# huster-wgm/SRCGAN

Hardware: AMD Instinct MI355X
Metric: paired SR-CycleGAN train images/sec at x4 256->1024 (higher is better)
Workload: dtype bf16; 1 GPU; Sat2Aerx4 paired G+D step (BASELINE configs[1]): 23-block RRDB generator + 3-layer PatchGAN, 3x256x256->3x1024x1024, batch 16/GPU; per_gpu_batch=16, global_batch=16, parallelism=dp1, gradient_exchange=none (1 rank)

## Files before the change

include/srcgan_amd.h:

```cpp
#ifndef SRCGAN_AMD_H
#define SRCGAN_AMD_H

#include <stddef.h>
#include <stdint.h>

#ifdef __cplusplus
extern "C" {
#endif

#define SRCGAN_F32 0
#define SRCGAN_BF16 1
#define SRCGAN_F16 2

int srcgan_version(void);
const char* srcgan_last_error(void);
int srcgan_dtype_size(int dtype);

int srcgan_nchw_f32_to_nhwc(const float* src, void* dst, int B, int C, int H, int W,
                            int cs, int dtype, void* stream);
int srcgan_nhwc_to_nchw_f32(const void* src, float* dst, int B, int C, int H, int W,
                            int cs, int coff, int dtype, void* stream);

size_t srcgan_packed_weight_bytes(int rows, int kdim, int ntaps, int dtype);
int srcgan_pack_weight(const float* w, void* wp, int rows, int kdim, int tys, int txs,
// ... 34 lines not shown
    int nsplit;
    long sr, sk, sty, stx, off;
    float alpha;
    int accumulate;
} srcgan_wgrad_desc;
size_t srcgan_conv_wgrad_slab_bytes(int Cout, int Cin, int kh, int kw, int nsplit);
int srcgan_conv_wgrad_nsplit(int B, int OH, int OW, int Cout, int Cin, int stride);
int srcgan_conv_wgrad(const srcgan_wgrad_desc* d, void* stream);

typedef struct srcgan_wgrad_seg { int g0, g1; float* grad; float* bias; int Cin; float alpha; } srcgan_wgrad_seg;
typedef struct srcgan_wgrad_dense_desc {
    const void* dy; const void* x; float* slab;
    int dtype;
    int B, H, W;
    int G, dy_cs, dy_coff;
    int C, x_cs, x_coff;
    int nseg;
    srcgan_wgrad_seg seg[8];
    int accumulate;
    long dy_plane, x_plane;
} srcgan_wgrad_dense_desc;
size_t srcgan_wgrad_dense_slab_bytes(int G, int C, int dtype, int B, int H, int W);
int srcgan_wgrad_dense(const srcgan_wgrad_dense_desc* d, void* stream);

int srcgan_col_reduce_blocks(long npix);
int srcgan_col_reduce(int mode, const void* a, int a_cs, int a_coff, const void* z, int z_cs, int z_coff,
                      const float* m, const float* rstd, long npix, int C, float scale,
                      float* out0, float* out1, float* scratch, int dtype, void* stream);

int srcgan_bn_finalize(const float* mean, const float* var, float* rstd, float* running_mean,
                       float* running_var, int64_t* num_batches_tracked, int C, long count,
                       float momentum, float eps, void* stream);
int srcgan_bn_eval_rstd(const float* running_var, float* rstd, int C, float eps, void* stream);
int srcgan_bn_apply_lrelu(const void* z, void* y, const float* mean, const float* rstd, const float* gamma,
                          const float* beta, long npix, int C, int cs, float slope, int dtype, void* stream);
int srcgan_bn_bwd_apply(const void* g, const void* z, void* dz, const float* mean, const float* rstd,
                        const float* gamma, const float* sum_g, const float* sum_gx, long npix, int C, int cs,
                        int dtype, void* stream);

int srcgan_add_inplace(void* y, int y_cs, int y_coff, const void* x, int x_cs, int x_coff,
                       const void* mz, int mz_cs, int mz_coff, float mslope, long npix, int C, int dtype, void* stream);
int srcgan_add_inplace_planes(void* y, int y_cs, int y_coff, long y_plane, const void* x, int x_cs, int x_coff, long x_plane,
                              const void* mz, int mz_cs, int mz_coff, long mz_plane, float mslope, long npix, int C,
                              int dtype, void* stream);

size_t srcgan_gn_scratch_floats(int B, int C);
// ... 382 lines not shown
```

srcgan_amd/_native.py:

```python
from __future__ import annotations

import ctypes as C
import os
from typing import Optional, Sequence

import torch

_HERE = os.path.dirname(os.path.abspath(__file__))
LIB_PATH = os.environ.get("SRCGAN_AMD_LIB") or os.path.join(_HERE, "lib", "libsrcgan_amd.so")

F32, BF16, F16 = 0, 1, 2
_DTYPES = {"fp32": F32, "f32": F32, "float32": F32, torch.float32: F32,
           "bf16": BF16, "bfloat16": BF16, torch.bfloat16: BF16,
           "fp16": F16, "f16": F16, "float16": F16, "half": F16, torch.float16: F16, F32: F32, BF16: BF16, F16: F16}
_default_dtype = _DTYPES[os.environ.get("SRCGAN_AMD_DTYPE", "fp32")]


def dtype_id(d) -> int:
    if d is None:
        return _default_dtype
    try:
        return _DTYPES[d]
    except KeyError:
        raise ValueError(f"unsupported compute dtype {d!r} (use 'fp32', 'bf16' or 'fp16')") from None
# ... 25 lines not shown
                ("sign_out", C.c_void_p), ("sign_in", C.c_void_p), ("npar", C.c_int), ("wpar_stride", C.c_long)]


class WgradDesc(C.Structure):
    _fields_ = [("dy", C.c_void_p), ("x", C.c_void_p), ("slab", C.c_void_p), ("grad", C.c_void_p), ("bias_grad", C.c_void_p),
                ("dtype", C.c_int), ("kh", C.c_int), ("kw", C.c_int), ("stride", C.c_int),
                ("B", C.c_int), ("H", C.c_int), ("W", C.c_int), ("Cin", C.c_int), ("x_cs", C.c_int), ("x_coff", C.c_int),
                ("OH", C.c_int), ("OW", C.c_int), ("Cout", C.c_int), ("dy_cs", C.c_int), ("dy_coff", C.c_int),
                ("pad_y", C.c_int), ("pad_x", C.c_int), ("nsplit", C.c_int),
                ("sr", C.c_long), ("sk", C.c_long), ("sty", C.c_long), ("stx", C.c_long), ("off", C.c_long),
                ("alpha", C.c_float), ("accumulate", C.c_int)]


class WgradSeg(C.Structure):
    _fields_ = [("g0", C.c_int), ("g1", C.c_int), ("grad", C.c_void_p), ("bias", C.c_void_p), ("Cin", C.c_int), ("alpha", C.c_float)]


class WgradDenseDesc(C.Structure):
    _fields_ = [("dy", C.c_void_p), ("x", C.c_void_p), ("slab", C.c_void_p), ("dtype", C.c_int),
                ("B", C.c_int), ("H", C.c_int), ("W", C.c_int),
                ("G", C.c_int), ("dy_cs", C.c_int), ("dy_coff", C.c_int),
                ("C", C.c_int), ("x_cs", C.c_int), ("x_coff", C.c_int),
                ("nseg", C.c_int), ("seg", WgradSeg * 8), ("accumulate", C.c_int), ("dy_plane", C.c_long), ("x_plane", C.c_long)]


class RddbCfg(C.Structure):
    _fields_ = [("in_ch", C.c_int), ("out_ch", C.c_int), ("up", C.c_int), ("nf", C.c_int), ("nb", C.c_int), ("gc", C.c_int),
                ("B", C.c_int), ("H", C.c_int), ("W", C.c_int), ("dtype", C.c_int), ("down", C.c_int), ("legacy", C.c_int)]


class NetOpts(C.Structure):
    _fields_ = [("wpack", C.c_void_p), ("pack", C.c_int), ("rrdb_lo", C.c_int), ("rrdb_hi", C.c_int), ("guard", C.c_void_p)]


class ResDeconvCfg(C.Structure):
    _fields_ = [("in_ch", C.c_int), ("out_ch", C.c_int), ("B", C.c_int), ("H", C.c_int), ("W", C.c_int), ("dtype", C.c_int),
                ("layers", C.c_int * 4), ("norm", C.c_int)]


class SrNetCfg(C.Structure):
    _fields_ = [(n, C.c_int) for n in ("kind", "in_ch", "out_ch", "up", "base", "B", "H", "W", "dtype", "nres")]


class SrDenseCfg(C.Structure):
    _fields_ = [(n, C.c_int) for n in ("kind", "in_ch", "out_ch", "B", "H", "W", "dtype", "growth", "num_blocks", "num_layers", "up")]

# ... 32 lines not shown


class NLayerDCfg(C.Structure):
    _fields_ = [("in_ch", C.c_int), ("ndf", C.c_int), ("n_layers", C.c_int),
                ("B", C.c_int), ("H", C.c_int), ("W", C.c_int), ("dtype", C.c_int), ("training", C.c_int), ("norm", C.c_int)]


_P, _I, _L, _F, _S = C.c_void_p, C.c_int, C.c_long, C.c_float, C.c_size_t
SIGNATURES = {
    "srcgan_version": (_I, []),
    "srcgan_last_error": (C.c_char_p, []),
    "srcgan_dtype_size": (_I, [_I]),
    "srcgan_nchw_f32_to_nhwc": (_I, [_P, _P, _I, _I, _I, _I, _I, _I, _P]),
    "srcgan_nhwc_to_nchw_f32": (_I, [_P, _P, _I, _I, _I, _I, _I, _I, _I, _P]),
    "srcgan_packed_weight_bytes": (_S, [_I, _I, _I, _I]),
    "srcgan_pack_weight": (_I, [_P, _P, _I, _I, _I, _I, _L, _L, _L, _L, _L, _I, _P]),
    "srcgan_pack_weight_part": (_I, [_P, _P, _I, _I, _I, _I, _L, _L, _L, _L, _L, _I, _I, _F, _I, _P]),
    "srcgan_conv_igemm": (_I, [C.POINTER(ConvDesc), _P]),
    "srcgan_conv_wgrad_slab_bytes": (_S, [_I, _I, _I, _I, _I]),
    "srcgan_conv_wgrad_nsplit": (_I, [_I, _I, _I, _I, _I, _I]),
    "srcgan_conv_wgrad": (_I, [C.POINTER(WgradDesc), _P]),
    "srcgan_wgrad_dense_slab_bytes": (_S, [_I, _I, _I, _I, _I, _I]),
    "srcgan_wgrad_dense": (_I, [C.POINTER(WgradDenseDesc), _P]),
    "srcgan_col_reduce_blocks": (_I, [_L]),
    "srcgan_col_reduce": (_I, [_I, _P, _I, _I, _P, _I, _I, _P, _P, _L, _I, _F, _P, _P, _P, _I, _P]),
    "srcgan_bn_finalize": (_I, [_P, _P, _P, _P, _P, _P, _I, _L, _F, _F, _P]),
    "srcgan_bn_eval_rstd": (_I, [_P, _P, _I, _F, _P]),
    "srcgan_bn_apply_lrelu": (_I, [_P, _P, _P, _P, _P, _P, _L, _I, _I, _F, _I, _P]),
    "srcgan_bn_bwd_apply": (_I, [_P, _P, _P, _P, _P, _P, _P, _P, _L, _I, _I, _I, _P]),
    "srcgan_add_inplace": (_I, [_P, _I, _I, _P, _I, _I, _P, _I, _I, _F, _L, _I, _I, _P]),
    "srcgan_add_inplace_planes": (_I, [_P, _I, _I, _L, _P, _I, _I, _L, _P, _I, _I, _L, _F, _L, _I, _I, _P]),
    "srcgan_gn_scratch_floats": (_S, [_I, _I]),
    "srcgan_gn_forward": (_I, [_P, _I, _P, _I, _P, _I, _P, _P, _P, _I, _L, _I, _I, _F, _I, _F, _I, _P, _P]),
    "srcgan_gn_backward": (_I, [_P, _I, _P, _I, _P, _I, _P, _P, _P, _I, _P, _I, _I, _P, _P, _I, _F, _I, _L, _I, _I, _I, _P, _P]),
    "srcgan_ca_scratch_floats": (_S, [_I, _L, _I]),
    "srcgan_ca_forward": (_I, [_P, _I, _P, _I, _P, _I, _P, _P, _P, _P, _P, _I, _L, _I, _I, _I, _P, _P]),
    "srcgan_ca_backward": (_I, [_P, _I, _P, _I, _P, _P, _P, _P, _I, _P, _I, _I, _P, _P, _P, _P, _I, _L, _I, _I, _I, _P, _P]),
    "srcgan_s2d_shift": (_I, [_P, _I, _P, _I, _I, _I, _I, _I, _I, _I, _I, _I, _I, _P]),
    "srcgan_d2s_shift": (_I, [_P, _I, _P, _I, _I, _I, _I, _I, _I, _I, _I, _I, _I, _I, _P]),
    "srcgan_prelu_forward": (_I, [_P, _I, _P, _P, _P, _I, _F, _P, _I, _I, _I, _I, _I, _I, _I, _I, _I, _I, _P]),
    "srcgan_prelu_scratch_floats": (_S, [_I, _I, _I, _I, _I]),
    "srcgan_prelu_backward": (_I, [_P, _I, _P, _I, _P, _P, _P, _I, _P, _I, _F, _I, _P, _P, _I, _I, _I, _I, _I, _I, _I, _I, _I, _P, _P]),
    "srcgan_reflect_pad_nhwc": (_I, [_P, _I, _P, _I, _I, _I, _I, _I, _I, _I, _P]),
    "srcgan_reflect_pad_bwd_nhwc": (_I, [_P, _I, _P, _I, _I, _I, _I, _I, _I, _I, _I, _P]),
    "srcgan_tanh_forward": (_I, [_P, _I, _P, _I, _L, _I, _I, _P]),
    "srcgan_tanh_backward": (_I, [_P, _I, _P, _I, _P, _I, _L, _I, _I, _I, _P]),
# ... 195 lines not shown
```

srcgan_amd/build.py:

```python
import glob
import os
import subprocess
import sys
from concurrent.futures import ThreadPoolExecutor

HERE = os.path.dirname(os.path.abspath(__file__))
CSRC = os.path.join(HERE, "csrc")
LIBDIR = os.path.join(HERE, "lib")
LIB = os.path.join(LIBDIR, "libsrcgan_amd.so")
SOURCES = ["conv_entry.hip", "conv_igemm.hip", "conv_par4.hip", "deconv_k3s2.hip", "conv3x3_dma.hip", "conv_wgrad.hip", "wgrad_dense.hip", "elementwise.hip", "class_losses.hip", "groupnorm.hip", "chan_attn.hip", "back_proj.hip", "reflect_pad.hip", "unet_skip.hip", "metrics.hip", "shift_select.hip", "scene_score.hip", "colour.hip", "tiles.hip", "vgg_loss.hip", "nets.hip", "oplist.hip"]
FLAGS = ["--offload-arch=gfx950", "-O3", "-std=c++17", "-fPIC", "-Wall", "-Wno-unused-function"]


def _hipcc():
    for c in (os.environ.get("HIPCC"), "/opt/rocm/bin/hipcc", "hipcc"):
        if c and (os.path.isabs(c) and os.path.exists(c) or not os.path.isabs(c)):
            return c
    raise RuntimeError("hipcc not found")


def _stale(target, deps):
    if not os.path.exists(target):
        return True
    t = os.path.getmtime(target)
    return any(os.path.getmtime(d) > t for d in deps)


def build(force=False, verbose=True):
    os.makedirs(LIBDIR, exist_ok=True)
    hipcc = _hipcc()
    headers = glob.glob(os.path.join(CSRC, "*.h")) + [os.path.join(HERE, "..", "include", "srcgan_amd.h")]
    objs, jobs = [], []
    for s in SOURCES:
# ... 23 lines not shown
```

srcgan_amd/csrc/nets.hip:

```cpp
#include "net_common.h"
#include <map>
#include <mutex>
#include <string>

int sg_zigzag_next() {
    static const bool zig = sg_env("SRCGAN_NO_ZIGZAG") == nullptr;
    static int flip = 0;
    const int rev = flip;
    flip ^= 1;
    return zig ? rev : 0;
}

namespace {
struct PackCache { std::vector<SgPackJob> host; SgPackJob* dev = nullptr; SgPackJob* pinned = nullptr; size_t cap = 0; hipEvent_t staged = nullptr; };
std::map<std::string, PackCache> g_pack_cache;
std::mutex g_pack_mutex;
}

int sg_pack_list_run(const std::vector<SgPackJob>& jobs, long nblk, void* wp_base, int dtype, const char* tag, const void* key_ptr, void* st,
                     const unsigned long long* guard) {
    if (jobs.empty()) return 0;
    int dev = 0;
    SG_HIP(hipGetDevice(&dev));
    char key[112];
    snprintf(key, sizeof(key), "%s:%d:%p:%d:%zu", tag, dev, key_ptr, dtype, jobs.size());
    std::lock_guard<std::mutex> lock(g_pack_mutex);
// ... 118 lines not shown
    for (int s = 0; s < P.nst; ++s) { for (int q = 0; q < 4; ++q) P.w_up_f[s][q] = pk(c->nf, c->nf, 1); P.w_up_d[s] = pk(c->nf, c->nf, 4); }
    P.w_last_f = pk(c->out_ch, c->nf, 9); P.w_last_d = pk(c->nf, P.out_cs, 9);
    for (int k = 0; k < P.nlw; ++k) { P.lw_f[k] = pk(c->nf, c->nf, 9); P.lw_d[k] = pk(c->nf, c->nf, 9); }
    P.w_rdb_d0 = wb.off;
    for (int i = 0; i < nrdb; ++i)
        for (int j = 0; j < 5; ++j) P.w_rdb_d[i * 5 + j] = pk(j == 0 ? c->nf : c->gc, c->nf + (4 - j) * c->gc, 9);
    P.w_rdb_dsz = wb.off - P.w_rdb_d0;
    P.wpack_bytes = wb.off + 256;
    int n = 0;
    P.p_first_w = n++; P.p_first_b = n++;
    P.p_dn0 = n; n += 2 * P.ndn;
    P.p_rdb0 = n; n += c->nb * 30;
    P.p_trunk_w = n++; P.p_trunk_b = n++;
    if (P.family == RDDB_SRDN) n += c->nb * 30;
    P.p_up0 = n;
    if (P.x2_tail) for (int k = 0; k < P.nlw; ++k) { P.p_lg[k] = n; n += 2; }
    else n += P.nst;
    P.p_last_w = n++;
    P.p_last_b = P.x2_tail ? n++ : -1;
    P.nparams = n;
    return 0;
}

struct RddbNames {
    size_t xin = 0, fea0 = 0, dn[5] = {}, T = 0, U[6] = {}, out = 0, tail[16] = {}, wpk = 0, total = 0;
    std::vector<size_t> A;
    size_t home = 0;
    bool rolling = false;
    size_t bm = 0; long bm_bytes = 0;
    size_t um = 0; long um_bytes = 0;
};

static void rddb_train_names(const srcgan_rddbnet_cfg* c, const RddbPlan& P, RddbNames& N) {
    const size_t e = P.esz, B = c->B, nf = c->nf;
    Bump b;
    N.xin = b.take(B * c->H * c->W * P.in_cs * e);
    if (P.ndn) N.fea0 = b.take(B * c->H * c->W * nf * e);
    for (int s = 0; s < P.ndn; ++s) N.dn[s] = b.take(B * (c->H >> (s + 1)) * (c->W >> (s + 1)) * nf * e);
    static const bool no_sign = sg_env("SRCGAN_NO_SIGNMASK") != nullptr || sg_env("SRCGAN_DMA_CFG") != nullptr;
    N.bm_bytes = (!no_sign && sg_is16(c->dtype) && c->gc == 32 && nf % 32 == 0 && P.family != RDDB_LEGACY) ? (long)B * P.Ht * P.Wt * 4 : 0;
    N.bm = align_up((size_t)P.nplane * P.plane_bytes, 256);
    const size_t szA = align_up(N.bm + 4 * (size_t)N.bm_bytes, 256);
    const size_t A0 = b.take(szA * P.ndense);
    N.A.resize(P.ndense);
    for (int r = 0; r < P.ndense; ++r) N.A[r] = A0 + (size_t)r * szA;
    N.T = b.take(B * P.Ht * P.Wt * nf * e);
    for (int s = 0; s <= P.nup; ++s) N.U[s] = b.take(B * (P.Ht << s) * (P.Wt << s) * nf * e);
    if (P.family == RDDB_SRDN) N.U[0] = N.T;
    for (int k = 0; k < P.ntail; ++k) N.tail[k] = b.take(B * P.tail[k].hout * P.tail[k].wout * nf * e);
    N.out = b.take(B * P.HO * P.WO * P.out_cs * e);
    N.um_bytes = (!no_sign && sg_is16(c->dtype) && nf == 64 && P.nst > 0 && P.family == RDDB_PLAIN) ? (long)B * P.HO * P.WO * 8 : 0;
    if (N.um_bytes) N.um = b.take((size_t)N.um_bytes);
    N.wpk = b.off;
    N.total = N.wpk + P.wpack_bytes;
}

static void rddb_infer_names(const srcgan_rddbnet_cfg* c, const RddbPlan& P, RddbNames& N) {
    const size_t e = P.esz, B = c->B, nf = c->nf;
    Bump b;
    N.rolling = true;
    N.xin = b.take(B * c->H * c->W * P.in_cs * e);
    if (P.ndn) {
        const size_t pp0 = b.take(B * c->H * c->W * nf * e);
        const size_t pp1 = P.ndn > 1 ? b.take(B * (c->H >> 1) * (c->W >> 1) * nf * e) : 0;
        N.fea0 = pp0;
        for (int s = 0; s < P.ndn; ++s) N.dn[s] = (s & 1) ? pp0 : pp1;
    }
    const size_t szA = align_up((size_t)P.nplane * P.plane_bytes, 256);
    size_t slot[3] = {0, 0, 0};
    for (int k = 0; k < 3 && k < P.ndense; ++k) slot[k] = b.take(szA);
    N.A.resize(P.ndense);
    int cur = 0, rrdb_in = 0;
    for (int r = 0; r < P.ndense; ++r) {
        if (r % 3 == 0) rrdb_in = cur;
// ... 27 lines not shown
struct RddbBwdPlan {
    size_t dout, dU[6], Pg[3], szP, dfea_dn[5], dxin, slab, colscr, total;
};
static void rddb_bwd_plan(const srcgan_rddbnet_cfg* c, const RddbPlan& P, RddbBwdPlan& Q) {
    const size_t e = P.esz, B = c->B;
    Bump b;
    Q.dout = b.take(B * P.HO * P.WO * P.out_cs * e);
    for (int s = 0; s <= P.nup; ++s) Q.dU[s] = b.take(B * (P.Ht << s) * (P.Wt << s) * c->nf * e);
    if (P.x2_tail) { Q.dU[1] = b.take(B * P.HO * P.WO * c->nf * e); Q.dU[2] = b.take(B * P.HO * P.WO * c->nf * e); }
    Q.szP = align_up((size_t)P.nplane * P.plane_bytes, 256);
    for (int i = 0; i < 3; ++i) Q.Pg[i] = b.take(Q.szP);
    for (int s = 0; s <= P.ndn; ++s) Q.dfea_dn[s] = b.take(B * (c->H >> s) * (c->W >> s) * c->nf * e);
    Q.dxin = b.take(B * c->H * c->W * P.in_cs * e);
    size_t slab = 0;
    auto mx = [&](size_t v) { if (v > slab) slab = v; };
    mx(wgrad_slab(c->B, c->H, c->W, c->nf, P.in_cs, 3, 3, 1));
    for (int k = 0; k < 5; ++k) mx(wgrad_slab(c->B, P.Ht, P.Wt, k < 4 ? c->gc : c->nf, c->nf + k * c->gc, 3, 3, 1));
    mx(wgrad_slab(c->B, P.Ht, P.Wt, c->nf, c->nf, 3, 3, 1));
    for (int s = 0; s < P.nup; ++s) mx(wgrad_slab(c->B, P.Ht << s, P.Wt << s, c->nf, c->nf, 2, 2, 2));
    for (int k = 0; k < P.ntail; ++k) if (P.tail[k].conv) mx(wgrad_slab(c->B, P.tail[k].hout, P.tail[k].wout, c->nf, c->nf, 3, 3, 1));
    for (int s = 0; s < P.ndn; ++s) mx(wgrad_slab(c->B, c->H >> (s + 1), c->W >> (s + 1), c->nf, c->nf, 3, 3, 2));
    mx(wgrad_slab(c->B, P.HO, P.WO, c->out_ch, c->nf, 3, 3, 1));
    mx(srcgan_wgrad_dense_slab_bytes(P.C, P.C, c->dtype, c->B, P.Ht, P.Wt));
    Q.slab = b.take(slab);
    const long maxpix = (long)B * (P.HO > c->H ? P.HO : c->H) * (P.WO > c->W ? P.WO : c->W);
    Q.colscr = b.take((size_t)2 * srcgan_col_reduce_blocks(maxpix) * P.C * sizeof(float));
    Q.total = b.off + 256;
}

}

extern "C" int srcgan_rddbnet_num_params(const srcgan_rddbnet_cfg* c) { RddbPlan P; if (rddb_plan(c, P)) return -1; return P.nparams; }
extern "C" int srcgan_rddbnet_num_rrdb(const srcgan_rddbnet_cfg* c) { RddbPlan P; if (rddb_plan(c, P)) return -1; return P.nrr; }
extern "C" size_t srcgan_rddbnet_wpack_bytes(const srcgan_rddbnet_cfg* c) { RddbPlan P; if (rddb_plan(c, P)) return 0; return P.wpack_bytes; }
extern "C" size_t srcgan_rddbnet_ws_bytes(const srcgan_rddbnet_cfg* c) {
    RddbPlan P; if (rddb_plan(c, P)) return 0;
    RddbNames N; rddb_train_names(c, P, N); return N.total;
}
extern "C" size_t srcgan_rddbnet_infer_ws_bytes(const srcgan_rddbnet_cfg* c) {
    RddbPlan P; if (rddb_plan(c, P)) return 0;
    RddbNames N; rddb_infer_names(c, P, N); return N.total;
}
extern "C" size_t srcgan_rddbnet_bwd_scratch_bytes(const srcgan_rddbnet_cfg* c) {
    RddbPlan P; if (rddb_plan(c, P)) return 0;
    RddbBwdPlan Q; rddb_bwd_plan(c, P, Q); return Q.total;
}
// ... 138 lines not shown
    RddbPlan P;
    SG_TRY(rddb_plan(c, P));
    RddbNames N;
    if (infer) rddb_infer_names(c, P, N); else rddb_train_names(c, P, N);
    return RddbCall(c, P, N, params, ws, opt, st).forward(x_nchw, y_nchw);
}

extern "C" int srcgan_rddbnet_forward_ex(const srcgan_rddbnet_cfg* c, const float* x_nchw, const float* const* params,
                                         void* ws, float* y_nchw, const srcgan_net_opts* opt, void* st) {
    return rddb_forward(c, false, x_nchw, params, ws, y_nchw, opt, st);
}

extern "C" int srcgan_rddbnet_infer(const srcgan_rddbnet_cfg* c, const float* x_nchw, const float* const* params, void* ws,
                                    float* y_nchw, const srcgan_net_opts* opt, void* st) {
    return rddb_forward(c, true, x_nchw, params, ws, y_nchw, opt, st);
}

extern "C" int srcgan_rddbnet_forward(const srcgan_rddbnet_cfg* c, const float* x_nchw, const float* const* params,
                                      void* ws, float* y_nchw, void* st) {
    return srcgan_rddbnet_forward_ex(c, x_nchw, params, ws, y_nchw, nullptr, st);
}

namespace {

struct RddbBwd : RddbCall {
    const RddbBwdPlan& Q;
    char* s8; float* const* grads;
    float* slab; float* colscr;
    const long npix_t;
    RddbBwd(const RddbCall& call, const RddbBwdPlan& Q_, void* scratch, float* const* grads_)
        : RddbCall(call), Q(Q_), s8((char*)scratch), grads(grads_), slab((float*)(s8 + Q_.slab)), colscr((float*)(s8 + Q_.colscr)),
          npix_t((long)B * H * W) {}
    TRef S_(size_t off, int cs) const { return tref(s8 + off, cs); }
    float* G(int idx) const { return grads[idx]; }
    TRef dout() const { return S_(Q.dout, P.out_cs); }
    TRef dU0() const { return S_(Q.dU[0], nf); }
    TRef Pg(int g) const { return tref(s8 + Q.Pg[g], P.kce, 0, P.plane_bytes); }
    int pack_dgrad(bool pack_dx) const;
    int output_plain() const;
    int output_tail() const;
    int trunk_entry() const;
    int rrdb_range(int r_lo, int r_hi) const;
    int input_side(float* dx_nchw) const;
};

int RddbBwd::pack_dgrad(bool pack_dx) const {
// ... 7 lines not shown
    if (P.family != RDDB_SRDN) packs.add(params[P.p_trunk_w], wp + P.w_trunk_d, nf, nf, 3, 3, L);
    SG_TRY(sg_fill_zero_guarded(wp + P.w_rdb_d0, P.w_rdb_dsz, pack_guard(opt), (hipStream_t)st));
    for (int r = 0; r < P.nrr * 3; ++r) {
        const float a5 = (r % 3 == 2) ? 0.04f : 0.2f;
        for (int j = 0; j < 5; ++j) {
            const int rows = j == 0 ? nf : gc, ss = j == 0 ? 0 : nf + (j - 1) * gc, ktot = nf + (4 - j) * gc;
            for (int m = 5; m > j; --m) {
                const int cin_m = nf + (m - 1) * gc, cout_m = m == 5 ? nf : gc;
                const int k_off = m == 5 ? 0 : nf + (4 - m) * gc;
                packs.add(params[P.prdb(r) + (m - 1) * 2], wp + P.w_rdb_d[r * 5 + j], rows, cout_m, 3, 3,
                                               9, (long)cin_m * 9, -3, -1, (long)ss * 9 + 8, k_off, ktot, m == 5 ? a5 : 1.f);
            }
        }
    }
    for (int s = 0; s < P.ndn; ++s) P.dn_dgrad().pack(packs, params[P.p_dn0 + 2 * s], wp, P.w_dn_d[s]);
    if (pack_dx) packs.add(params[P.p_first_w], wp + P.w_first_d, c->in_ch, nf, 3, 3, lay_dgrad_s1(c->in_ch, 3, 3));
    return packs.run((std::string(P.tag) + (pack_dx ? "_bwd_dx" : "_bwd")).c_str(), params[0], st, pack_guard(opt));
}

int RddbBwd::output_plain() const {
    TRef Ul = T_(N.U[P.nup], nf);
    if (G(P.p_last_w))
        SG_TRY(wgrad_call(dt, dout(), P.HO, P.WO, c->out_ch, Ul, B, P.HO, P.WO, nf, 3, 3, 1, 1, 1, lay_fwd(nf, 3, 3), 1.f, slab, G(P.p_last_w), st));
    {
        Conv cv(dt, 3, 3, 1);
        cv.in(dout(), B, P.HO, P.WO, P.out_cs).w(wp + P.w_last_d).out(S_(Q.dU[P.nup], nf), P.HO, P.WO, nf).pad(1, 1);
        if (P.nup > 0) {
            if (N.um_bytes) { cv.sign_in(w8 + N.um); cv.d.mslope = 0.2f; }
            else cv.mask(Ul, 0);
        }
        SG_TRY(cv.run(st));
    }
    for (int s = P.nup - 1; s >= 0; --s) {
        const int h = H << s, w = W << s;
        TRef dHR = S_(Q.dU[s + 1], nf), Us = T_(N.U[s], nf);
        if (G(P.p_up0 + s))
            SG_TRY(wgrad_call(dt, Us, h, w, nf, dHR, B, 2 * h, 2 * w, nf, 2, 2, 2, 0, 0, WLayout{(long)nf * 4, 4, 2, 1, 0}, 1.f, slab, G(P.p_up0 + s), st));
        Conv cv(dt, 2, 2, 2);
        cv.in(dHR, B, 2 * h, 2 * w, nf).w(wp + P.w_up_d[s]).out(S_(Q.dU[s], nf), h, w, nf).pad(0, 0);
        if (s > 0) cv.mask(Us, 0);
        SG_TRY(cv.run(st));
    }
    return 0;
}

int RddbBwd::output_tail() const {
    TRef tin = P.family == RDDB_LEGACY ? Abuf(0) : T_(N.U[0], nf);
    auto obuf = [&](int k) { return k < 0 ? tin : T_(N.tail[k], nf); };
    TRef Fl = obuf(P.ntail - 1);
    if (G(P.p_last_w))
        SG_TRY(wgrad_call(dt, dout(), P.HO, P.WO, c->out_ch, Fl, B, P.HO, P.WO, nf, 3, 3, 1, 1, 1, lay_fwd(nf, 3, 3), 1.f, slab, G(P.p_last_w), st, G(P.p_last_b)));
    else if (G(P.p_last_b)) SG_TRY(bias_grad(dt, dout(), (long)B * P.HO * P.WO, c->out_ch, 1.f, G(P.p_last_b), colscr, st));
    int pp = 0;
    auto nextbuf = [&](int k_in) { if (k_in < 0) return dU0(); pp ^= 1; return S_(Q.dU[1 + pp], nf); };
    TRef dcur = nextbuf(P.ntail - 1);
    {
// ... 139 lines not shown
    int r_lo = 0, r_hi = P.nrr;
    if (opt && opt->rrdb_hi > 0) { r_lo = opt->rrdb_lo; r_hi = opt->rrdb_hi; }
    SG_REQUIRE(r_lo >= 0 && r_lo <= r_hi && r_hi <= P.nrr, "srcgan_rddbnet_backward: RRDB range [%d,%d) outside [0,%d)", r_lo, r_hi, P.nrr);
    SG_REQUIRE(P.nrr > 0 || (r_lo == 0), "srcgan_rddbnet_backward: a network without a trunk has one phase");
    const bool first_phase = r_hi == P.nrr, last_phase = r_lo == 0;
    const RddbBwd K(RddbCall(c, P, N, params, ws, opt, st), Q, scratch, grads);
    if (first_phase) {
        const bool pack_dx = dx_nchw || (opt && opt->wpack);
        if (K.do_pack) SG_TRY(K.pack_dgrad(pack_dx));
        SG_TRY(srcgan_nchw_f32_to_nhwc(dy_nchw, K.dout().p, c->B, c->out_ch, P.HO, P.WO, P.out_cs, c->dtype, st));
        SG_TRY(P.x2_tail ? K.output_tail() : K.output_plain());
        if (P.nrr) SG_TRY(K.trunk_entry());
    }
    SG_TRY(K.rrdb_range(r_lo, r_hi));
    if (last_phase) SG_TRY(K.input_side(dx_nchw));
    return 0;
}

extern "C" int srcgan_rddbnet_backward(const srcgan_rddbnet_cfg* c, const float* dy_nchw, const float* const* params,
                                       void* ws, void* scratch, float* const* grads, float* dx_nchw, void* st) {
    return srcgan_rddbnet_backward_ex(c, dy_nchw, params, ws, scratch, grads, dx_nchw, nullptr, st);
}

namespace {
enum DPost { D_LRELU, D_BNORM, D_INORM, D_FINAL };
struct DLayer {
    int k, stride, pad;
    int H, W, Cin, in_cs;
    int OH, OW, Cout, out_cs;
    DPost post;
    bool folded;
    int pw, pb, pg, pbeta, bn_idx;
    size_t X, Y, Z, stat;
    size_t wf, wf_bytes, wd[4], wd_bytes;
    bool normed() const { return post == D_BNORM || post == D_INORM; }
    S2Dgrad s2() const { return S2Dgrad{k, pad, Cin, Cout}; }
};
struct DPlan {
    int esz, L, nparams, cmax;
    bool inorm;
    DLayer y[8];
    size_t colscr, gnscr, wpk, total;
    bool s2d() const { return y[0].folded; }
};

static int d_plan(const srcgan_nlayerd_cfg* c, DPlan& P) {
// ... 264 lines not shown
```

Measured before the change: 119.8 images/s.

## Fuse generator tail backward: last-conv dgrad with upsample deconv dgrad and wgrad

Adds a fused tail backward path for the RRDB generator's output stage. The last 3x3 conv's input gradient (with sign-mask LeakyReLU) is recomputed on chip from a halo tile and fed straight into the 2x2 stride-2 upsample's dgrad and wgrad through MFMA, so the full-resolution 64-channel dU2 tensor is never written or read at 1024x1024. In exchange the 3x3 dgrad is computed twice (once per kernel), and the wgrad goes through a per-workgroup slab plus a separate reduction. It is on by default for bf16/fp16 plain RRDB nets with the sign mask and can be disabled with SRCGAN_NO_TAIL_FUSE.

Result: no change. 121.0 images/s, median of 6 (+1.0%).

```diff
diff --git a/include/srcgan_amd.h b/include/srcgan_amd.h
--- a/include/srcgan_amd.h
+++ b/include/srcgan_amd.h
@@ -80,6 +80,18 @@
 } srcgan_wgrad_dense_desc;
 size_t srcgan_wgrad_dense_slab_bytes(int G, int C, int dtype, int B, int H, int W);
 int srcgan_wgrad_dense(const srcgan_wgrad_dense_desc* d, void* stream);
+
+typedef struct srcgan_tail_bwd_desc {
+    const void* dout; const void* um; const void* u1;
+    const float* w_last; const float* w_up;
+    void* wpack; void* du2; void* du1;
+    float* slab; float* grad_up;
+    int B, h, w, out_ch, dtype, mask_in, fused;
+    float mslope;
+} srcgan_tail_bwd_desc;
+size_t srcgan_tail_bwd_wpack_bytes(int dtype);
+size_t srcgan_tail_bwd_slab_bytes(int B, int h, int w);
+int srcgan_tail_bwd(const srcgan_tail_bwd_desc* d, void* stream);
 
 int srcgan_col_reduce_blocks(long npix);
 int srcgan_col_reduce(int mode, const void* a, int a_cs, int a_coff, const void* z, int z_cs, int z_coff,
diff --git a/srcgan_amd/_native.py b/srcgan_amd/_native.py
--- a/srcgan_amd/_native.py
+++ b/srcgan_amd/_native.py
@@ -71,6 +71,13 @@
                 ("G", C.c_int), ("dy_cs", C.c_int), ("dy_coff", C.c_int),
                 ("C", C.c_int), ("x_cs", C.c_int), ("x_coff", C.c_int),
                 ("nseg", C.c_int), ("seg", WgradSeg * 8), ("accumulate", C.c_int), ("dy_plane", C.c_long), ("x_plane", C.c_long)]
+
+
+class TailBwdDesc(C.Structure):
+    _fields_ = [("dout", C.c_void_p), ("um", C.c_void_p), ("u1", C.c_void_p), ("w_last", C.c_void_p), ("w_up", C.c_void_p),
+                ("wpack", C.c_void_p), ("du2", C.c_void_p), ("du1", C.c_void_p), ("slab", C.c_void_p), ("grad_up", C.c_void_p),
+                ("B", C.c_int), ("h", C.c_int), ("w", C.c_int), ("out_ch", C.c_int), ("dtype", C.c_int), ("mask_in", C.c_int),
+                ("fused", C.c_int), ("mslope", C.c_float)]
 
 
 class RddbCfg(C.Structure):
@@ -149,6 +156,9 @@
     "srcgan_conv_wgrad": (_I, [C.POINTER(WgradDesc), _P]),
     "srcgan_wgrad_dense_slab_bytes": (_S, [_I, _I, _I, _I, _I, _I]),
     "srcgan_wgrad_dense": (_I, [C.POINTER(WgradDenseDesc), _P]),
+    "srcgan_tail_bwd_wpack_bytes": (_S, [_I]),
+    "srcgan_tail_bwd_slab_bytes": (_S, [_I, _I, _I]),
+    "srcgan_tail_bwd": (_I, [C.POINTER(TailBwdDesc), _P]),
     "srcgan_col_reduce_blocks": (_I, [_L]),
     "srcgan_col_reduce": (_I, [_I, _P, _I, _I, _P, _I, _I, _P, _P, _L, _I, _F, _P, _P, _P, _I, _P]),
     "srcgan_bn_finalize": (_I, [_P, _P, _P, _P, _P, _P, _I, _L, _F, _F, _P]),
diff --git a/srcgan_amd/build.py b/srcgan_amd/build.py
--- a/srcgan_amd/build.py
+++ b/srcgan_amd/build.py
@@ -8,7 +8,7 @@
 CSRC = os.path.join(HERE, "csrc")
 LIBDIR = os.path.join(HERE, "lib")
 LIB = os.path.join(LIBDIR, "libsrcgan_amd.so")
-SOURCES = ["conv_entry.hip", "conv_igemm.hip", "conv_par4.hip", "deconv_k3s2.hip", "conv3x3_dma.hip", "conv_wgrad.hip", "wgrad_dense.hip", "elementwise.hip", "class_losses.hip", "groupnorm.hip", "chan_attn.hip", "back_proj.hip", "reflect_pad.hip", "unet_skip.hip", "metrics.hip", "shift_select.hip", "scene_score.hip", "colour.hip", "tiles.hip", "vgg_loss.hip", "nets.hip", "oplist.hip"]
+SOURCES = ["conv_entry.hip", "conv_igemm.hip", "conv_par4.hip", "deconv_k3s2.hip", "conv3x3_dma.hip", "conv_wgrad.hip", "wgrad_dense.hip", "tail_bwd.hip", "elementwise.hip", "class_losses.hip", "groupnorm.hip", "chan_attn.hip", "back_proj.hip", "reflect_pad.hip", "unet_skip.hip", "metrics.hip", "shift_select.hip", "scene_score.hip", "colour.hip", "tiles.hip", "vgg_loss.hip", "nets.hip", "oplist.hip"]
 FLAGS = ["--offload-arch=gfx950", "-O3", "-std=c++17", "-fPIC", "-Wall", "-Wno-unused-function"]
 
 
diff --git a/srcgan_amd/csrc/nets.hip b/srcgan_amd/csrc/nets.hip
--- a/srcgan_amd/csrc/nets.hip
+++ b/srcgan_amd/csrc/nets.hip
@@ -1,7 +1,9 @@
 #include "net_common.h"
+#include "tail_bwd.h"
 #include <map>
 #include <mutex>
 #include <string>
+#include <stdlib.h>
 
 int sg_zigzag_next() {
     static const bool zig = sg_env("SRCGAN_NO_ZIGZAG") == nullptr;
@@ -166,6 +168,15 @@
     return 0;
 }
 
+static bool rddb_um_on(const srcgan_rddbnet_cfg* c, const RddbPlan& P) {
+    static const bool no_sign = sg_env("SRCGAN_NO_SIGNMASK") != nullptr || sg_env("SRCGAN_DMA_CFG") != nullptr;
+    return !no_sign && sg_is16(c->dtype) && c->nf == 64 && P.nst > 0 && P.family == RDDB_PLAIN;
+}
+static bool rddb_tail_fused(const srcgan_rddbnet_cfg* c, const RddbPlan& P) {
+    static const bool off = getenv("SRCGAN_NO_TAIL_FUSE") != nullptr;
+    return !off && !P.x2_tail && P.nup >= 1 && rddb_um_on(c, P) && P.out_cs == 8 && c->out_ch <= 4;
+}
+
 struct RddbNames {
     size_t xin = 0, fea0 = 0, dn[5] = {}, T = 0, U[6] = {}, out = 0, tail[16] = {}, wpk = 0, total = 0;
     std::vector<size_t> A;
@@ -193,7 +204,7 @@
     if (P.family == RDDB_SRDN) N.U[0] = N.T;
     for (int k = 0; k < P.ntail; ++k) N.tail[k] = b.take(B * P.tail[k].hout * P.tail[k].wout * nf * e);
     N.out = b.take(B * P.HO * P.WO * P.out_cs * e);
-    N.um_bytes = (!no_sign && sg_is16(c->dtype) && nf == 64 && P.nst > 0 && P.family == RDDB_PLAIN) ? (long)B * P.HO * P.WO * 8 : 0;
+    N.um_bytes = rddb_um_on(c, P) ? (long)B * P.HO * P.WO * 8 : 0;
     if (N.um_bytes) N.um = b.take((size_t)N.um_bytes);
     N.wpk = b.off;
     N.total = N.wpk + P.wpack_bytes;
@@ -267,6 +278,7 @@
     for (int s = 0; s < P.ndn; ++s) mx(wgrad_slab(c->B, c->H >> (s + 1), c->W >> (s + 1), c->nf, c->nf, 3, 3, 2));
     mx(wgrad_slab(c->B, P.HO, P.WO, c->out_ch, c->nf, 3, 3, 1));
     mx(srcgan_wgrad_dense_slab_bytes(P.C, P.C, c->dtype, c->B, P.Ht, P.Wt));
+    if (rddb_tail_fused(c, P)) mx(sg_tail_bwd_slab_bytes(c->B, P.HO / 2, P.WO / 2));
     Q.slab = b.take(slab);
     const long maxpix = (long)B * (P.HO > c->H ? P.HO : c->H) * (P.WO > c->W ? P.WO : c->W);
     Q.colscr = b.take((size_t)2 * srcgan_col_reduce_blocks(maxpix) * P.C * sizeof(float));
@@ -451,6 +463,34 @@
 }
 
 namespace {
+
+struct TailStage {
+    int dt, B, h, w; float mslope; bool mask_in;
+    TRef dout; const void* um; TRef U1; const char* w_last_d; const char* w_up_d; TRef dU2, dU1; float* slab; float* gW;
+};
+static int tail_stage_fused(const TailStage& t, void* st) {
+    SG_REQUIRE(t.dout.cs == 8 && t.U1.cs == 64 && t.dU1.cs == 64 && !t.dout.coff && !t.U1.coff && !t.dU1.coff && !t.U1.plane && !t.dU1.plane,
+               "tail backward: operands must be plain NHWC (8 / 64 channels)");
+    TailBwdP p;
+    memset(&p, 0, sizeof(p));
+    p.dout = t.dout.p; p.um = t.um; p.u1 = t.U1.p; p.w_last_d = t.w_last_d; p.w_up_d = t.w_up_d; p.du1 = t.dU1.p; p.slab = t.slab; p.grad = t.gW;
+    p.B = t.B; p.h = t.h; p.w = t.w; p.mask_in = t.mask_in; p.mslope = t.mslope;
+    if (t.gW) SG_TRY(sg_tail_bwd_wgrad(p, t.dt, (hipStream_t)st));
+    return sg_tail_bwd_dgrad(p, t.dt, (hipStream_t)st);
+}
+static int tail_stage_unfused(const TailStage& t, void* st) {
+    const int HO = 2 * t.h, WO = 2 * t.w;
+    Conv cl(t.dt, 3, 3, 1);
+    cl.in(t.dout, t.B, HO, WO, 8).w(t.w_last_d).out(t.dU2, HO, WO, 64).pad(1, 1).sign_in(t.um);
+    cl.d.mslope = t.mslope;
+    SG_TRY(cl.run(st));
+    if (t.gW)
+        SG_TRY(wgrad_call(t.dt, t.U1, t.h, t.w, 64, t.dU2, t.B, HO, WO, 64, 2, 2, 2, 0, 0, WLayout{256, 4, 2, 1, 0}, 1.f, t.slab, t.gW, st));
+    Conv cv(t.dt, 2, 2, 2);
+    cv.in(t.dU2, t.B, HO, WO, 64).w(t.w_up_d).out(t.dU1, t.h, t.w, 64).pad(0, 0);
+    if (t.mask_in) { cv.mask(t.U1, 0); cv.d.mslope = t.mslope; }
+    return cv.run(st);
+}
 
 struct RddbBwd : RddbCall {
     const RddbBwdPlan& Q;
@@ -504,7 +544,16 @@
     TRef Ul = T_(N.U[P.nup], nf);
     if (G(P.p_last_w))
         SG_TRY(wgrad_call(dt, dout(), P.HO, P.WO, c->out_ch, Ul, B, P.HO, P.WO, nf, 3, 3, 1, 1, 1, lay_fwd(nf, 3, 3), 1.f, slab, G(P.p_last_w), st));
-    {
+    int s_top = P.nup - 1;
+    if (rddb_tail_fused(c, P)) {
+        const int s = P.nup - 1;
+        TailStage t;
+        t.dt = dt; t.B = B; t.h = H << s; t.w = W << s; t.mslope = 0.2f; t.mask_in = s > 0;
+        t.dout = dout(); t.um = w8 + N.um; t.U1 = T_(N.U[s], nf); t.w_last_d = wp + P.w_last_d; t.w_up_d = wp + P.w_up_d[s];
+        t.dU2 = TNULL; t.dU1 = S_(Q.dU[s], nf); t.slab = slab; t.gW = G(P.p_up0 + s);
+        SG_TRY(tail_stage_fused(t, st));
+        s_top = s - 1;
+    } else {
         Conv cv(dt, 3, 3, 1);
         cv.in(dout(), B, P.HO, P.WO, P.out_cs).w(wp + P.w_last_d).out(S_(Q.dU[P.nup], nf), P.HO, P.WO, nf).pad(1, 1);
         if (P.nup > 0) {
@@ -513,7 +562,7 @@
         }
         SG_TRY(cv.run(st));
     }
-    for (int s = P.nup - 1; s >= 0; --s) {
+    for (int s = s_top; s >= 0; --s) {
         const int h = H << s, w = W << s;
         TRef dHR = S_(Q.dU[s + 1], nf), Us = T_(N.U[s], nf);
         if (G(P.p_up0 + s))
@@ -699,6 +748,31 @@
     return srcgan_rddbnet_backward_ex(c, dy_nchw, params, ws, scratch, grads, dx_nchw, nullptr, st);
 }
 
+static size_t tail_wpack_last(int dtype) { return align_up(srcgan_packed_weight_bytes(64, 8, 9, dtype), 256); }
+extern "C" size_t srcgan_tail_bwd_wpack_bytes(int dtype) {
+    return sg_is16(dtype) ? tail_wpack_last(dtype) + align_up(srcgan_packed_weight_bytes(64, 64, 4, dtype), 256) : 0;
+}
+extern "C" size_t srcgan_tail_bwd_slab_bytes(int B, int h, int w) {
+    if (B <= 0 || h <= 0 || w <= 0) return 0;
+    return std::max(sg_tail_bwd_slab_bytes(B, h, w), wgrad_slab(B, h, w, 64, 64, 2, 2, 2));
+}
+extern "C" int srcgan_tail_bwd(const srcgan_tail_bwd_desc* d, void* st) {
+    SG_REQUIRE(d && d->dout && d->um && d->u1 && d->w_last && d->w_up && d->wpack && d->du1 && (d->fused || d->du2) && (!d->grad_up || d->slab),
+               "srcgan_tail_bwd: null pointer");
+    SG_REQUIRE(sg_is16(d->dtype) && d->B > 0 && d->h > 0 && d->w > 0 && d->out_ch >= 1 && d->out_ch <= 4, "srcgan_tail_bwd: 16-bit dtypes, out_ch in 1..4");
+    SG_REQUIRE(((uintptr_t)d->wpack % 256) == 0, "srcgan_tail_bwd: wpack must be 256-byte aligned");
+    char* wp = (char*)d->wpack;
+    PackList packs(d->dtype, wp);
+    packs.add(d->w_last, wp, 64, d->out_ch, 3, 3, lay_dgrad_s1(64, 3, 3));
+    packs.add(d->w_up, wp + tail_wpack_last(d->dtype), 64, 64, 2, 2, 256, 4, 2, 1, 0);
+    SG_TRY(packs.run("tail_bwd", d->w_last, st));
+    TailStage t;
+    t.dt = d->dtype; t.B = d->B; t.h = d->h; t.w = d->w; t.mslope = d->mslope; t.mask_in = d->mask_in != 0;
+    t.dout = tref((void*)d->dout, 8); t.um = d->um; t.U1 = tref((void*)d->u1, 64); t.w_last_d = wp; t.w_up_d = wp + tail_wpack_last(d->dtype);
+    t.dU2 = tref(d->du2, 64); t.dU1 = tref(d->du1, 64); t.slab = d->slab; t.gW = d->grad_up;
+    return d->fused ? tail_stage_fused(t, st) : tail_stage_unfused(t, st);
+}
+
 namespace {
 enum DPost { D_LRELU, D_BNORM, D_INORM, D_FINAL };
 struct DLayer {
diff --git a/srcgan_amd/csrc/tail_bwd.h b/srcgan_amd/csrc/tail_bwd.h
--- /dev/null
+++ b/srcgan_amd/csrc/tail_bwd.h
@@ -0,0 +1,20 @@
+#pragma once
+#include "common.h"
+
+constexpr int TAIL_WG_ELEMS = 64 * 64 * 4;
+constexpr int TAIL_MAX_WG = 512;
+
+struct TailBwdP {
+    const void* dout; const void* um; const void* u1; const void* w_last_d; const void* w_up_d;
+    void* du1; float* slab; float* grad;
+    int B, h, w, mask_in;
+    float mslope;
+    int tiles_x, tiles_y;
+};
+static inline size_t sg_tail_bwd_slab_bytes(int B, int h, int w) {
+    long n = (long)B * cdiv(h, 16) * cdiv(w, 16);
+    if (n > TAIL_MAX_WG) n = TAIL_MAX_WG;
+    return (size_t)n * TAIL_WG_ELEMS * sizeof(float);
+}
+int sg_tail_bwd_dgrad(const TailBwdP& p, int dtype, hipStream_t st);
+int sg_tail_bwd_wgrad(const TailBwdP& p, int dtype, hipStream_t st);
diff --git a/srcgan_amd/csrc/tail_bwd.hip b/srcgan_amd/csrc/tail_bwd.hip
--- /dev/null
+++ b/srcgan_amd/csrc/tail_bwd.hip
@@ -0,0 +1,377 @@
+#include "tail_bwd.h"
+#include "launch.h"
+
+namespace {
+
+constexpr int TL = 16;
+constexpr int HW_ = 2 * TL + 2;
+constexpr int NHALO = HW_ * HW_;
+constexpr int NTHR = 512;
+constexpr int HIT = (NHALO + NTHR - 1) / NTHR;
+
+struct UnitPos { int b, gy0, gx0; };
+
+__device__ __forceinline__ UnitPos unit_pos(const TailBwdP& p, int u) {
+    UnitPos o;
+    o.gx0 = (u % p.tiles_x) * TL; u /= p.tiles_x;
+    o.gy0 = (u % p.tiles_y) * TL; o.b = u / p.tiles_y;
+    return o;
+}
+
+__device__ __forceinline__ void halo_fetch(const TailBwdP& p, const UnitPos& o, int tid, u32x2 (&v)[HIT]) {
+    const int HO = 2 * p.h, WO = 2 * p.w;
+#pragma unroll
+    for (int it = 0; it < HIT; ++it) {
+        const int i = it * NTHR + tid, hy = i / HW_, hx = i - hy * HW_;
+        const int Y = 2 * o.gy0 - 1 + hy, X = 2 * o.gx0 - 1 + hx;
+        const bool ok = i < NHALO && (unsigned)Y < (unsigned)HO && (unsigned)X < (unsigned)WO;
+        u32x2 z = {0u, 0u};
+        v[it] = ok ? *(const u32x2*)((const char*)p.dout + (((long)o.b * HO + Y) * WO + X) * 16) : z;
+    }
+}
+__device__ __forceinline__ void halo_put(u32x2* halo, int tid, const u32x2 (&v)[HIT]) {
+#pragma unroll
+    for (int it = 0; it < HIT; ++it) {
+        const int i = it * NTHR + tid;
+        if (i < NHALO) halo[i] = v[it];
+    }
+}
+
+struct TapOff { int o[3][2]; };
+__device__ __forceinline__ TapOff tap_offsets(int h) {
+    TapOff t;
+#pragma unroll
+    for (int j = 0; j < 3; ++j)
+#pragma unroll
+        for (int i = 0; i < 2; ++i) {
+            const int t0 = 4 * j + i, t1 = 4 * j + 2 + i;
+            const int o0 = t0 < 9 ? (t0 / 3) * HW_ + t0 % 3 : -1, o1 = t1 < 9 ? (t1 / 3) * HW_ + t1 % 3 : -1;
+            t.o[j][i] = h ? o1 : o0;
+        }
+    return t;
+}
+__device__ __forceinline__ bf16x8 px_frag(const u32x2* halo, int base, int o0, int o1) {
+    u32x2 z = {0u, 0u};
+    const u32x2 lo = o0 >= 0 ? halo[base + o0] : z, hi = o1 >= 0 ? halo[base + o1] : z;
+    u32x4 f = {lo[0], lo[1], hi[0], hi[1]};
+    return __builtin_bit_cast(bf16x8, f);
+}
+template <typename T>
+__device__ __forceinline__ bf16x8 wlast_frag(const T* wl, int row, int j, int h) {
+    u32x2 z = {0u, 0u}, v[2];
+#pragma unroll
+    for (int i = 0; i < 2; ++i) {
+        const int t0 = 4 * j + i, t1 = 4 * j + 2 + i;
+        const int t = h ? t1 : t0;
+        v[i] = t < 9 ? *(const u32x2*)(wl + ((long)t * 64 + row) * 32) : z;
+    }
+    u32x4 f = {v[0][0], v[0][1], v[1][0], v[1][1]};
+    return __builtin_bit_cast(bf16x8, f);
+}
+template <typename T>
+__device__ __forceinline__ bf16x8 chain_frag(const float (&v)[16], int s) {
+    typedef __attribute__((ext_vector_type(8))) T v8;
+    v8 o;
+#pragma unroll
+    for (int i = 0; i < 8; ++i) o[i] = from_f<T>(v[8 * s + i]);
+    return __builtin_bit_cast(bf16x8, o);
+}
+
+__device__ __forceinline__ float mask_factor(unsigned word, unsigned pos, float slope) {
+    const unsigned sel = (unsigned)__builtin_amdgcn_sbfe((int)word, pos, 1u);
+    return __builtin_bit_cast(float, (sel & 0x3f800000u) | (~sel & __builtin_bit_cast(unsigned, slope)));
+}
+
+__device__ __forceinline__ void unit_range(int nunits, int& u0, int& u_hi, int& gw) {
+    const int xcd = blockIdx.x & 7, jw = blockIdx.x >> 3;
+    gw = (gridDim.x + 7 - xcd) >> 3;
+    const int u8 = (nunits + 7) >> 3, u_lo = xcd * u8;
+    u_hi = (u_lo + u8 < nunits) ? u_lo + u8 : nunits;
+    u0 = u_lo + jw;
+}
+
+template <typename T>
+__global__ __launch_bounds__(NTHR) void tail_dgrad_k(const TailBwdP p) {
+    __shared__ u32x2 halo[NHALO];
+    __shared__ u32x4 wu[4 * 4 * 2 * 64];
+    const int tid = threadIdx.x, lane = tid & 63, r = lane & 31, h = lane >> 5;
+    const int wave = __builtin_amdgcn_readfirstlane(tid >> 6);
+    int u, u_hi, gw;
+    unit_range(p.tiles_x * p.tiles_y * p.B, u, u_hi, gw);
+    if (u >= u_hi) return;
+    for (int e = tid; e < 4 * 64 * 16; e += NTHR) {
+        const int co4 = e & 15, ci = (e >> 4) & 63, q = e >> 10;
+        const int j = co4 >> 2, rem4 = co4 & 3, hh = rem4 & 1;
+        const u32x2 v = *(const u32x2*)((const T*)p.w_up_d + ((long)((co4 >> 3) * 4 + q) * 64 + ci) * 32 + (co4 & 7) * 4);
+        *(u32x2*)((char*)wu + ((((q * 4 + j) * 2 + hh) * 64 + ci) * 16 + (rem4 >> 1) * 8)) = v;
+    }
+    bf16x8 wl[2][3];
+#pragma unroll
+    for (int mt = 0; mt < 2; ++mt)
+#pragma unroll
+        for (int j = 0; j < 3; ++j) wl[mt][j] = wlast_frag<T>((const T*)p.w_last_d, 32 * mt + r, j, h);
+    const TapOff to = tap_offsets(h);
+    const int ly = 2 * wave + (r >> 4), lx = r & 15;
+    const int base0 = 2 * ly * HW_ + 2 * lx;
+    const int HO = 2 * p.h, WO = 2 * p.w;
+
+    UnitPos o = unit_pos(p, u);
+    u32x2 hv[HIT], uzn[8];
+    unsigned long long smn[4], sm[4];
+    unsigned zb = 0;
+    auto fetch = [&](const UnitPos& f) {
+        halo_fetch(p, f, tid, hv);
+        const int gy = f.gy0 + ly, gx = f.gx0 + lx;
+        const bool in = gy < p.h && gx < p.w;
+#pragma unroll
+        for (int q = 0; q < 4; ++q)
+            smn[q] = in ? ((const unsigned long long*)p.um)[((long)f.b * HO + 2 * gy + (q >> 1)) * WO + 2 * gx + (q & 1)] : 0ull;
+        if (p.mask_in) {
+            const T* up = (const T*)p.u1 + (((long)f.b * p.h + gy) * p.w + gx) * 64 + 4 * h;
+            const u32x2 z = {0u, 0u};
+#pragma unroll
+            for (int i = 0; i < 8; ++i) uzn[i] = in ? *(const u32x2*)(up + 8 * i) : z;
+        }
+    };
+    auto settle = [&]() {
+        typedef __attribute__((ext_vector_type(4))) T v4;
+#pragma unroll
+        for (int q = 0; q < 4; ++q) sm[q] = smn[q];
+        zb = 0;
+        if (p.mask_in) {
+#pragma unroll
+            for (int i = 0; i < 8; ++i) {
+                const v4 z = __builtin_bit_cast(v4, uzn[i]);
+#pragma unroll
+                for (int t = 0; t < 4; ++t) zb |= (to_f(z[t]) > 0.f ? 1u : 0u) << (4 * i + t);
+            }
+        }
+    };
+    fetch(o);
+    for (; u < u_hi; u += gw) {
+        __syncthreads();
+        halo_put(halo, tid, hv);
+        settle();
+        __syncthreads();
+        const UnitPos c = o;
+        if (u + gw < u_hi) { o = unit_pos(p, u + gw); fetch(o); }
+        const int gy = c.gy0 + ly, gx = c.gx0 + lx;
+        const bool inimg = gy < p.h && gx < p.w;
+        f32x16 acc[2];
+#pragma unroll
+        for (int m = 0; m < 2; ++m)
+#pragma unroll
+            for (int i = 0; i < 16; ++i) acc[m][i] = 0.f;
+#pragma unroll
+        for (int q = 0; q < 4; ++q) {
+            const int base = base0 + (q >> 1) * HW_ + (q & 1);
+            f32x16 d1[2];
+#pragma unroll
+            for (int mt = 0; mt < 2; ++mt)
+#pragma unroll
+                for (int i = 0; i < 16; ++i) d1[mt][i] = 0.f;
+#pragma unroll
+            for (int j = 0; j < 3; ++j) {
+                const bf16x8 b = px_frag(halo, base, to.o[j][0], to.o[j][1]);
+                d1[0] = sg_mfma16<T>(wl[0][j], b, d1[0]);
+                d1[1] = sg_mfma16<T>(wl[1][j], b, d1[1]);
+            }
+            bf16x8 bf[2][2];
+            const unsigned long long smh = sm[q] >> (4 * h);
+#pragma unroll
+            for (int mt = 0; mt < 2; ++mt) {
+                const unsigned word = mt ? (unsigned)(smh >> 32) : (unsigned)smh;
+                float v[16];
+#pragma unroll
+                for (int i = 0; i < 16; ++i)
+                    v[i] = d1[mt][i] * mask_factor(word, 8 * (i >> 2) + (i & 3), p.mslope);
+                bf[mt][0] = chain_frag<T>(v, 0);
+                bf[mt][1] = chain_frag<T>(v, 1);
+            }
+#pragma unroll
+            for (int j = 0; j < 4; ++j)
+#pragma unroll
+                for (int m = 0; m < 2; ++m) {
+                    const bf16x8 a = __builtin_bit_cast(bf16x8, wu[((q * 4 + j) * 2 + h) * 64 + 32 * m + r]);
+                    acc[m] = sg_mfma16<T>(a, bf[j >> 1][j & 1], acc[m]);
+                }
+        }
+        if (inimg) {
+            const long px = ((long)c.b * p.h + gy) * p.w + gx;
+            T* yp = (T*)p.du1 + px * 64;
+#pragma unroll
+            for (int m = 0; m < 2; ++m)
+#pragma unroll
+                for (int g = 0; g < 4; ++g) {
+                    const int ci0 = 32 * m + 8 * g + 4 * h;
+                    float v[4];
+#pragma unroll
+                    for (int t = 0; t < 4; ++t) v[t] = acc[m][4 * g + t];
+                    if (p.mask_in) {
+#pragma unroll
+                        for (int t = 0; t < 4; ++t) v[t] *= ((zb >> (4 * (4 * m + g) + t)) & 1u) ? 1.f : p.mslope;
+                    }
+                    store4<T>(yp + ci0, v);
+                }
+        }
+    }
+}
+
+constexpr int UIT = TL * TL * 8 / NTHR;
+constexpr int MIT = 4 * TL * TL / NTHR;
+
+template <typename T>
+__global__ __launch_bounds__(NTHR) void tail_wgrad_k(const TailBwdP p) {
+    __shared__ u32x2 halo[NHALO];
+    __shared__ unsigned long long sm[4 * TL * TL];
+    __shared__ u32x4 ut[8 * 2 * 2 * 64];
+    const int tid = threadIdx.x, lane = tid & 63, r = lane & 31, h = lane >> 5;
+    const int wave = __builtin_amdgcn_readfirstlane(tid >> 6);
+    const int q = wave >> 1, c2 = wave & 1, pa = q >> 1, pb = q & 1;
+    int u, u_hi, gw;
+    unit_range(p.tiles_x * p.tiles_y * p.B, u, u_hi, gw);
+    f32x16 acc[2];
+#pragma unroll
+    for (int m = 0; m < 2; ++m)
+#pragma unroll
+        for (int i = 0; i < 16; ++i) acc[m][i] = 0.f;
+    if (u < u_hi) {
+        bf16x8 wl[3];
+#pragma unroll
+        for (int j = 0; j < 3; ++j) wl[j] = wlast_frag<T>((const T*)p.w_last_d, 32 * c2 + r, j, h);
+        const TapOff to = tap_offsets(h);
+        const int HO = 2 * p.h, WO = 2 * p.w;
+        const int cobyte = (32 * c2 + r) >> 3, cobit = r & 7;
+        const int sw[2] = {r ^ (r >> 3), 32 + (r ^ (4 + (r >> 3)))};
+
+        u32x2 hv[HIT];
+        u32x4 uv[UIT];
+        unsigned long long mv[MIT];
+        auto fetch = [&](const UnitPos& o) {
+            halo_fetch(p, o, tid, hv);
+#pragma unroll
+            for (int it = 0; it < UIT; ++it) {
+                const int e = it * NTHR + tid, px = e >> 3, gy = o.gy0 + (px >> 4), gx = o.gx0 + (px & 15);
+                u32x4 z = {0u, 0u, 0u, 0u};
+                uv[it] = (gy < p.h && gx < p.w) ? *(const u32x4*)((const T*)p.u1 + (((long)o.b * p.h + gy) * p.w + gx) * 64 + (e & 7) * 8) : z;
+            }
+#pragma unroll
+            for (int it = 0; it < MIT; ++it) {
+                const int e = it * NTHR + tid, Y = 2 * o.gy0 + (e >> 5), X = 2 * o.gx0 + (e & 31);
+                mv[it] = (Y < HO && X < WO) ? ((const unsigned long long*)p.um)[((long)o.b * HO + Y) * WO + X] : 0ull;
+            }
+        };
+        auto put = [&]() {
+            halo_put(halo, tid, hv);
+#pragma unroll
+            for (int it = 0; it < UIT; ++it) {
+                const int e = it * NTHR + tid, px = e >> 3, ci0 = (e & 7) * 8;
+                const int pt = px >> 5, rr = px & 31, j = rr >> 4, rem = rr & 15, hh = (rem >> 2) & 1, s = (rem >> 3) * 4 + (rem & 3);
+                unsigned short* dst = (unsigned short*)ut + ((((pt * 2 + j) * 2 + hh) * 64 + ci0) * 8 + s);
+#pragma unroll
+                for (int k = 0; k < 8; ++k) dst[(k ^ (e & 7)) * 8] = (unsigned short)(uv[it][k >> 1] >> ((k & 1) * 16));
+            }
+#pragma unroll
+            for (int it = 0; it < MIT; ++it) sm[it * NTHR + tid] = mv[it];
+        };
+        UnitPos o = unit_pos(p, u);
+        fetch(o);
+        for (; u < u_hi; u += gw) {
+            __syncthreads();
+            put();
+            __syncthreads();
+            if (u + gw < u_hi) { o = unit_pos(p, u + gw); fetch(o); }
+#pragma unroll 1
+            for (int pt = 0; pt < 8; ++pt) {
+                const int base = (2 * (2 * pt + (r >> 4)) + pa) * HW_ + 2 * (r & 15) + pb;
+                f32x16 d1;
+#pragma unroll
+                for (int i = 0; i < 16; ++i) d1[i] = 0.f;
+#pragma unroll
+                for (int j = 0; j < 3; ++j) d1 = sg_mfma16<T>(px_frag(halo, base, to.o[j][0], to.o[j][1]), wl[j], d1);
+                float v[16];
+#pragma unroll
+                for (int i = 0; i < 16; ++i) {
+                    const int rr = 8 * (i >> 2) + 4 * h + (i & 3);
+                    const int Y = 2 * (2 * pt + (rr >> 4)) + pa, X = 2 * (rr & 15) + pb;
+                    const unsigned mb = ((const unsigned char*)sm)[(Y * 32 + X) * 8 + cobyte];
+                    v[i] = d1[i] * mask_factor(mb, cobit, p.mslope);
+                }
+                const bf16x8 b0 = chain_frag<T>(v, 0), b1 = chain_frag<T>(v, 1);
+#pragma unroll
+                for (int m = 0; m < 2; ++m) {
+                    acc[m] = sg_mfma16<T>(__builtin_bit_cast(bf16x8, ut[((pt * 2 + 0) * 2 + h) * 64 + sw[m]]), b0, acc[m]);
+                    acc[m] = sg_mfma16<T>(__builtin_bit_cast(bf16x8, ut[((pt * 2 + 1) * 2 + h) * 64 + sw[m]]), b1, acc[m]);
+                }
+            }
+        }
+    }
+    float* sl = p.slab + (size_t)blockIdx.x * TAIL_WG_ELEMS;
+#pragma unroll
+    for (int m = 0; m < 2; ++m)
+#pragma unroll
+        for (int i = 0; i < 16; ++i) {
+            const int ci = 32 * m + 8 * (i >> 2) + 4 * h + (i & 3), co = 32 * c2 + r;
+            sl[(ci * 64 + co) * 4 + q] = acc[m][i];
+        }
+}
+
+__global__ __launch_bounds__(256) void tail_wgrad_reduce_k(const float* __restrict__ slab, int nwg, float* __restrict__ grad) {
+    __shared__ float red[4][64];
+    const int el = threadIdx.x & 63, sl = threadIdx.x >> 6, e = blockIdx.x * 64 + el;
+    float a0 = 0.f, a1 = 0.f, a2 = 0.f, a3 = 0.f;
+    int sp = sl;
+    for (; sp + 12 < nwg; sp += 16) {
+        a0 += slab[(size_t)sp * TAIL_WG_ELEMS + e];
+        a1 += slab[(size_t)(sp + 4) * TAIL_WG_ELEMS + e];
+        a2 += slab[(size_t)(sp + 8) * TAIL_WG_ELEMS + e];
+        a3 += slab[(size_t)(sp + 12) * TAIL_WG_ELEMS + e];
+    }
+    for (; sp < nwg; sp += 4) a0 += slab[(size_t)sp * TAIL_WG_ELEMS + e];
+    red[sl][el] = (a0 + a1) + (a2 + a3);
+    __syncthreads();
+    if (sl == 0) grad[e] = (red[0][el] + red[1][el]) + (red[2][el] + red[3][el]);
+}
+
+static int tail_grid(const TailBwdP& p, TailBwdP& q, int per_cu, long cap, int& nwg) {
+    int dev = 0;
+    SG_TRY(sg_current_device(dev));
+    const int ncu = sg_cu_count(dev);
+    if (!ncu) return 1;
+    q = p;
+    q.tiles_x = cdiv(p.w, TL); q.tiles_y = cdiv(p.h, TL);
+    const long nunits = (long)q.tiles_x * q.tiles_y * p.B;
+    SG_REQUIRE(nunits < (1L << 30), "tail backward: too many tiles");
+    long n = (long)ncu * per_cu;
+    if (n > cap) n = cap;
+    if (n > nunits) n = nunits;
+    nwg = (int)n;
+    return 0;
+}
+
+}
+
+int sg_tail_bwd_dgrad(const TailBwdP& p, int dtype, hipStream_t st) {
+    SG_REQUIRE(sg_is16(dtype) && p.dout && p.um && p.u1 && p.du1 && p.w_last_d && p.w_up_d && p.B > 0 && p.h > 0 && p.w > 0, "tail backward: bad arguments");
+    TailBwdP q; int nwg = 0;
+    SG_TRY(tail_grid(p, q, 1, 1L << 20, nwg));
+    const double px = (double)p.B * p.h * p.w;
+    const int tok = sg_prof_start(dtype == SRCGAN_F16 ? "tail_dgrad<f16>" : "tail_dgrad<bf16>", 2.0 * px * 4 * 64 * (48 + 64), px * (4 * 24 + 128 * (p.mask_in ? 2 : 1)), st);
+    sg_dtype_dispatch16(dtype, [&](auto t) { hipLaunchKernelGGL(tail_dgrad_k<decltype(t)>, dim3((unsigned)nwg), dim3(NTHR), 0, st, q); return 0; });
+    sg_prof_stop(tok, st);
+    SG_LAUNCH_CHECK();
+    return 0;
+}
+
+int sg_tail_bwd_wgrad(const TailBwdP& p, int dtype, hipStream_t st) {
+    SG_REQUIRE(sg_is16(dtype) && p.dout && p.um && p.u1 && p.slab && p.grad && p.w_last_d && p.B > 0 && p.h > 0 && p.w > 0, "tail backward: bad arguments");
+    TailBwdP q; int nwg = 0;
+    SG_TRY(tail_grid(p, q, 1, TAIL_MAX_WG, nwg));
+    const double px = (double)p.B * p.h * p.w;
+    const int tok = sg_prof_start(dtype == SRCGAN_F16 ? "tail_wgrad<f16>" : "tail_wgrad<bf16>", 2.0 * px * 4 * 64 * (48 + 64), px * (4 * 24 + 128), st);
+    sg_dtype_dispatch16(dtype, [&](auto t) { hipLaunchKernelGGL(tail_wgrad_k<decltype(t)>, dim3((unsigned)nwg), dim3(NTHR), 0, st, q); return 0; });
+    hipLaunchKernelGGL(tail_wgrad_reduce_k, dim3(TAIL_WG_ELEMS / 64), dim3(256), 0, st, (const float*)p.slab, nwg, p.grad);
+    sg_prof_stop(tok, st);
+    SG_LAUNCH_CHECK();
+    return 0;
+}
```
